# imaginateit/csm-train-pytorch

Measured on AMD Instinct MI355X. Metric: train tokens/sec (text+audio) CSM-1B bf16 seq2048, higher is better.
Workload: dtype bf16

## Files before the change

### csm-train-pytorch_amd/csm/engine.py

```python
from __future__ import annotations

import math
import numbers
from contextlib import contextmanager
from typing import Dict, List, Optional

import torch

from .hip import ops

BF16 = torch.bfloat16
F32 = torch.float32
import os as _os
FUSE_SWIGLU = _os.environ.get("CSM_FUSE_SWIGLU", "1") == "1"
FUSE_ROPE_BWD = _os.environ.get("CSM_FUSE_ROPE_BWD", "1") == "1"
FUSE_ROPE_FWD = _os.environ.get("CSM_FUSE_ROPE_FWD", "1") == "1"
PAIR_DX_DW = int(_os.environ.get("CSM_PAIR_DX_DW", "0"))
GROUP_ATTN_DW = _os.environ.get("CSM_GROUP_ATTN_DW", "1") == "1"
DEFER_ATTN_DW = int(_os.environ.get("CSM_DEFER_ATTN_DW", "3"))
DEFER_NORM_DW = _os.environ.get("CSM_DEFER_NORM_DW", "1") == "1"
ROWS_ON_HOST = _os.environ.get("CSM_ROWS_ON_HOST", "1") == "1"
EMB_KEYSORT = _os.environ.get("CSM_EMB_KEYSORT", "1") == "1"
DECODE_POS_HOST = _os.environ.get("CSM_DECODE_POS_HOST", "1") == "1"
LORA_FUSE = _os.environ.get("CSM_LORA_FUSE", "1") != "0"


def _refuse_stack(lo, where: str):
    if getattr(lo, "n_adapters", 1) > 1:
        raise ValueError(f"{where} takes one adapter set, and model.lora stacks {lo.n_adapters}: export one first "
                         "(state = model.lora.export(a), then LoRABank.add / generate_batch(adapters=[...]) / row_lora(model, state))")


def adapter_rows(adapter_ids, B: int, S: int, n_adapters: int, segment_lengths=None) -> torch.Tensor:
    ids = torch.as_tensor(adapter_ids).detach().to("cpu")
    if ids.is_floating_point() or ids.dtype == torch.bool:
        raise ValueError(f"adapter_ids must be integers, got {ids.dtype}")
    ids = ids.to(torch.int64)
# ... 650 lines not shown
        dh0 = self.backbone.backward(dhid, B, S, tr["backbone"], 1.0, on_layer_done=self.grad_hook, acc=acc["backbone"], seg=s.get("seg"),
                                    sel=s.get("sel"))
        if train_embeddings:
            self._embedding_backward(s, dh0, dseq if (dec is not None and s["aw"] != 0.0) else None)
        if self.grad_hook is not None:
            self.grad_hook("embeddings", -1)

    def _embedding_backward(self, s, dh0, dseq):
        m, a = self.m, self.m.args
        dev = m.device
        K, V = a.audio_num_codebooks, a.audio_vocab_size
        TV = a.text_vocab_size
        n_rows = TV + K * V
        tk, mk = s["tk"], s["mk"]
        M = tk.shape[0]
        ck = ("embbwd", M, K, V, TV)
        c = self._consts.get(ck)
        if c is None:
            slot = torch.arange(K + 1, device=dev)
            c = self._consts[ck] = dict(off=torch.where(slot < K, TV + slot * V, torch.zeros_like(slot)),
                                        src=torch.arange(M, device=dev).unsqueeze(1).expand(M, K + 1).reshape(-1).contiguous())
        rows = torch.where(mk.bool(), tk + c["off"], torch.full_like(tk, n_rows)).reshape(-1)
        src = c["src"]
        n_src = M
        if dseq is not None:
            codes, N = s["dec"]["codes"], s["dec"]["N"]
            dk = ("embbwd_dec", M, N, K, V, TV)
            d = self._consts.get(dk)
            if d is None:
                d = self._consts[dk] = dict(off=TV + torch.arange(K - 1, device=dev) * V,
                                            src=(M + torch.arange(N, device=dev).unsqueeze(1) * K + torch.arange(1, K, device=dev)).reshape(-1))
            rows = torch.cat([rows, (codes[:, :K - 1] + d["off"]).reshape(-1)])
            src = torch.cat([src, d["src"]])
            n_src = M + N * K
        if n_src <= (1 << 20) and EMB_KEYSORT:
            key = torch.sort((rows << 20) | src).values
            rows_s, src_s = key >> 20, key & ((1 << 20) - 1)
        else:
            order = torch.argsort(rows, stable=True)
            rows_s, src_s = rows[order].contiguous(), src[order].contiguous()
        ops.embed_bwd_sorted(rows_s, src_s, dh0, dseq,
                             m.block("text_embeddings.weight", True), m.block("audio_embeddings.weight", True))

    @torch.no_grad()
    def hidden_states(self, tokens: torch.Tensor, masks: torch.Tensor) -> torch.Tensor:
        m, a = self.m, self.m.args
        B, S, K1 = tokens.shape
        M = B * S
        tk = tokens.reshape(M, K1).to(device=m.device, dtype=torch.int64).contiguous()
        mk = masks.reshape(M, K1).to(device=m.device, dtype=torch.uint8).contiguous()
        h0 = torch.empty(M, m.bb.embed_dim, dtype=BF16, device=m.device)
        self._need()
        ops.embed_fwd(tk, mk, m.block("text_embeddings.weight"), m.block("audio_embeddings.weight"), h0, a.audio_vocab_size)
        return self.backbone.forward(h0, B, S, False).view(B, S, -1)

    @torch.no_grad()
    def generate_frame(self, tokens, tokens_mask, input_pos, temperature, topk, noise=None, adapters=None, top_p=None,
# ... 921 lines not shown
```

### csm-train-pytorch_amd/csm/hip/__init__.py

```python
import ctypes as C
import os

_HERE = os.path.dirname(os.path.abspath(__file__))
LIB_PATH = os.environ.get("CSM_HIP_LIB") or os.path.join(_HERE, "libcsm_hip.so")


class CsmHipError(RuntimeError):
    pass


if not os.path.exists(LIB_PATH):
    raise ImportError(
        f"{LIB_PATH} is missing: build it with `python __graft_entry__.py build` (or `make -C csm-train-pytorch_amd/csrc`). "
        "The CSM MI355X path has no fallback implementation."
    )

lib = C.CDLL(LIB_PATH)

_p, _i, _f, _ll = C.c_void_p, C.c_int, C.c_float, C.c_longlong

_SIGS = {
    "csm_abi_version": ([], _i),
    "csm_last_error": ([], C.c_char_p),
    "csm_device_check": ([_i], _i),
# ... 23 lines not shown
    "csm_colsum_rows_bf16": ([_p, _i, _ll, _i, _p, _i, _p], _i),
    "csm_rope": ([_p, _p, _p, _ll, _i, _i, _i, _i, _i, _p], _i),
    "csm_set_attn_variant": ([_i], _i),
    "csm_attn_last_dkv_kernel": ([], _i),
    "csm_attn64_set_debug": ([_p], _i),
    "csm_set_decode_tuning": ([_i, _i], _i),
    "csm_attn_fwd": ([_p, _p, _p, _i, _i, _i, _i, _i, _p], _i),
    "csm_attn_bwd": ([_p, _p, _p, _p, _p, _p, _i, _i, _i, _i, _i, _p], _i),
    "csm_attn_bwd_rope": ([_p, _p, _p, _p, _p, _p, _p, _i, _i, _i, _i, _i, _p], _i),
    "csm_attn_fwd_seg": ([_p, _p, _p, _p, _i, _i, _i, _i, _i, _p], _i),
    "csm_attn_bwd_seg": ([_p, _p, _p, _p, _p, _p, _p, _p, _i, _i, _i, _i, _i, _p], _i),
    "csm_swiglu_fwd": ([_p, _p, _ll, _i, _p], _i),
    "csm_swiglu_bwd": ([_p, _p, _p, _ll, _i, _p], _i),
    "csm_embed_fwd": ([_p, _p, _p, _p, _p, _ll, _i, _i, _i, _p], _i),
    "csm_embed_bwd_sorted": ([_p, _p, _ll, _p, _p, _ll, _p, _p, _ll, _ll, _i, _p], _i),
    "csm_rows_add_bf16": ([_p, _p, _p, _ll, _i, _i, _p], _i),
    "csm_rows_take_bf16": ([_p, _p, _p, _ll, _i, _p], _i),
    "csm_decoder_input_fwd": ([_p, _p, _p, _p, _p, _ll, _i, _i, _i, _p], _i),
    "csm_ce_fwd_bwd": ([_p, _p, _p, _p, _ll, _i, _i, _i, _f, _p], _i),
    "csm_reduce_sum_f32": ([_p, _ll, _f, _p, _p], _i),
    "csm_sumsq_blocks": ([], _i),
    "csm_sumsq_bf16": ([_p, _ll, _p, _p], _i),
    "csm_clip_coef": ([_p, _i, _f, _p, _p], _i),
    "csm_adamw_step": ([_p, _p, _p, _p, _p, _ll, _f, _f, _f, _f, _f, _i, _p, _f, _i, _p], _i),
    "csm_adamw_step_split": ([_p, _p, _p, _p, _p, _ll, _f, _f, _f, _f, _f, _i, _p, _f, _i, _p], _i),
    "csm_adamw_step_live": ([_p, _p, _p, _p, _p, _ll, _f, _f, _f, _f, _f, _i, _p, _f, _i, _p, _p], _i),
    "csm_adamw_step_split_live": ([_p, _p, _p, _p, _p, _ll, _f, _f, _f, _f, _f, _i, _p, _f, _i, _p, _p], _i),
    "csm_set_adamw_blocks": ([_i], _i),
    "csm_gemv_bf16": ([_p, _p, _p, _p, _i, _i, _i, _i, _i, _i, _i, _p], _i),
    "csm_gemv_last_kernel": ([], C.c_char_p),
# ... 82 lines not shown
```

### csm-train-pytorch_amd/csm/hip/ops.py

```python
import ctypes
import math
from typing import Optional

import torch

from . import CsmHipError, check, lib

BF16 = torch.bfloat16


def _stream() -> int:
    return torch.cuda.current_stream().cuda_stream


def _ptr(t: Optional[torch.Tensor]) -> Optional[int]:
    return None if t is None else t.data_ptr()


def _mat(t: torch.Tensor, dtype=BF16):
    assert t.is_cuda and t.dtype == dtype and t.dim() == 2 and t.stride(1) == 1, (t.dtype, t.shape, t.stride())
    return t.data_ptr(), t.shape[0], t.shape[1], t.stride(0)


def _pin(pin):
# ... 294 lines not shown

def swiglu_bwd(gu, dout, dgu):
    M, F2 = gu.shape
    check(lib.csm_swiglu_bwd(gu.data_ptr(), dout.data_ptr(), dgu.data_ptr(), M, F2 // 2, _stream()), "csm_swiglu_bwd")
    return dgu


def embed_fwd(tokens, mask_u8, text_emb, audio_emb, out, audio_vocab):
    M, K1 = tokens.shape
    assert tokens.dtype == torch.int64 and mask_u8.dtype == torch.uint8 and tokens.is_contiguous() and mask_u8.is_contiguous()
    check(lib.csm_embed_fwd(tokens.data_ptr(), mask_u8.data_ptr(), text_emb.data_ptr(), audio_emb.data_ptr(), out.data_ptr(),
                            M, K1 - 1, out.shape[1], audio_vocab, _stream()), "csm_embed_fwd")
    return out


def embed_bwd_sorted(sorted_rows, src_index, dh, dseq, g_text, g_audio):
    assert sorted_rows.dtype == torch.int64 and src_index.dtype == torch.int64 and sorted_rows.is_contiguous() and src_index.is_contiguous()
    check(lib.csm_embed_bwd_sorted(sorted_rows.data_ptr(), src_index.data_ptr(), sorted_rows.numel(), dh.data_ptr(), _ptr(dseq),
                                   dh.shape[0], g_text.data_ptr(), g_audio.data_ptr(), g_text.shape[0],
                                   g_text.shape[0] + g_audio.shape[0], dh.shape[1], _stream()), "csm_embed_bwd_sorted")


def rows_add_bf16(dst, rows_i32, src, src_stride_rows):
    check(lib.csm_rows_add_bf16(dst.data_ptr(), rows_i32.data_ptr(), src.data_ptr(), rows_i32.numel(), int(src_stride_rows),
                                dst.shape[1], _stream()), "csm_rows_add_bf16")


def rows_take_bf16(table, rows_i32, out):
    assert rows_i32.dtype == torch.int32 and rows_i32.is_contiguous() and out.is_contiguous() and out.shape == (rows_i32.numel(), table.shape[1])
    check(lib.csm_rows_take_bf16(table.data_ptr(), rows_i32.data_ptr(), out.data_ptr(), rows_i32.numel(), table.shape[1], _stream()),
# ... 13 lines not shown
    R, ldl = logits_f32.shape[0], logits_f32.stride(0)
    assert logits_f32.dtype == torch.float32 and targets.dtype == torch.int64 and targets.is_contiguous()
    ldd = dlogits.stride(0) if dlogits is not None else 0
    check(lib.csm_ce_fwd_bwd(logits_f32.data_ptr(), targets.data_ptr(), loss_rows.data_ptr(), _ptr(dlogits), R, V, ldl, ldd,
                             float(grad_scale), _stream()), "csm_ce_fwd_bwd")


def reduce_sum(x_f32, out_f32, scale=1.0):
    check(lib.csm_reduce_sum_f32(x_f32.data_ptr(), x_f32.numel(), float(scale), out_f32.data_ptr(), _stream()), "csm_reduce_sum_f32")


def sumsq_blocks() -> int:
    return lib.csm_sumsq_blocks()


def sumsq_bf16(g, partials):
    check(lib.csm_sumsq_bf16(g.data_ptr(), g.numel(), partials.data_ptr(), _stream()), "csm_sumsq_bf16")


def clip_coef(partials, max_norm, norm_and_coef):
    check(lib.csm_clip_coef(partials.data_ptr(), partials.numel(), float(max_norm), norm_and_coef.data_ptr(), _stream()), "csm_clip_coef")


ADAMW_BLOCK = 2048


def _live_ptr(block_live, n):
    assert block_live.dtype == torch.uint8 and block_live.is_contiguous() and block_live.numel() == -(-n // ADAMW_BLOCK)
    return block_live.data_ptr()


def adamw_step(master, m, v, param, grad, lr, beta1, beta2, eps, wd, step, norm_and_coef=None, grad_mul=1.0, zero_grad=False, *,
# ... 473 lines not shown
```

### csm-train-pytorch_amd/csm/models/model.py

```python
from __future__ import annotations

import math
from collections import OrderedDict
from dataclasses import dataclass
from typing import Dict, List, Optional, Tuple

import torch
import torch.nn as nn

from ..hip import ops, require_device

BF16 = torch.bfloat16


@dataclass
class StackConfig:
    embed_dim: int
    num_layers: int
    num_heads: int
    num_kv_heads: int
    intermediate_dim: int
    max_seq_len: int = 2048
    norm_eps: float = 1e-5
    rope_base: float = 500_000.0
# ... 143 lines not shown
        super().__init__()
        self.args = args
        self.bb: StackConfig = FLAVORS[args.backbone_flavor]()
        self.dc: StackConfig = FLAVORS[args.decoder_flavor]()
        self.vocab_pad = _pad64(args.audio_vocab_size)
        self._slots: Dict[str, _Slot] = OrderedDict()
        self._groups: Dict[str, Tuple[int, int]] = {}
        self._plan()
        self._device = torch.device("cpu")
        self.arena: Optional[torch.Tensor] = None
        self.grad_arena: Optional[torch.Tensor] = None
        self.lora = None
        self.acoustic_mode = "off"
        self.acoustic_fraction = 1.0 / 16.0
        self.grad_state = {"backbone": "zero", "decoder": "zero", "embeddings": "zero", "other": "zero"}
        self.target_ignore_index = None
        self._tables: Dict[str, torch.Tensor] = {}
        self._engine = None
        self._init_seed = seed
        self._fp32_source = None
        self.use_kv_cache = True
        self.use_hip_graph = True
        self._decode_weights = "bf16"
        self.trainable = {"backbone": True, "decoder": True, "embeddings": True, "other": True}
        if device is not None:
            self.to(device)

    @property
    def decode_weights(self) -> str:
        return self._decode_weights
# ... 69 lines not shown
        stack("decoder", self.dc)
        out["text_embeddings.weight"] = blk("text_embeddings.weight")
        out["audio_embeddings.weight"] = blk("audio_embeddings.weight")
        out["projection.weight"] = blk("projection.weight")
        out["codebook0_head.weight"] = blk("codebook0_head.padded")[:a.audio_vocab_size]
        out["audio_head"] = blk("audio_head.padded")[:, :, :a.audio_vocab_size]
        return out

    def block(self, name: str, grad: bool = False) -> torch.Tensor:
        s = self._slots[name]
        src = self.grad_arena if grad else self.arena
        return src[s.offset:s.offset + s.numel].view(s.shape)

    def group_range(self, group: str) -> Tuple[int, int]:
        return self._groups[group]

    def to(self, *args, **kwargs):
        device = kwargs.get("device", None)
        for a in args:
            if isinstance(a, (str, torch.device)):
                device = a
        if device is None:
            return self
        device = torch.device(device)
        if device.type != "cuda":
            raise RuntimeError("csm (MI355X build): the model lives on a gfx950 GPU; there is no CPU execution path")
        require_device(device.index or 0)
        if device.index is None:
            device = torch.device("cuda", torch.cuda.current_device())
        old = self.arena
        self.arena = torch.zeros(self._numel, dtype=BF16, device=device)
        if old is not None:
            self.arena.copy_(old)
        self.grad_arena = None
        self._device = device
        self._bind()
        if old is None:
            self.reset_parameters(self._init_seed)
        self._tables = {}
        self._engine = None
        return self

    def cuda(self, device=None):
        return self.to(torch.device("cuda", device if device is not None else torch.cuda.current_device()))

    def _bind(self):
        for name, view in self._views(self.arena).items():
            mod, _, leaf = name.rpartition(".")
            holder = self
# ... 123 lines not shown
```

### csm-train-pytorch_amd/csm/training/dp.py

```python
import os
from typing import Callable, Dict, List, Optional, Tuple

import torch
import torch.distributed as dist


def init_distributed(backend: Optional[str] = None) -> Tuple[int, int, int]:
    rank, world = int(os.environ.get("RANK", 0)), int(os.environ.get("WORLD_SIZE", 1))
    local = int(os.environ.get("LOCAL_RANK", 0))
    os.environ.setdefault("HSA_ENABLE_IPC_MODE_LEGACY", "0")
    if world > 1 and not dist.is_initialized():
        if torch.cuda.is_available():
            torch.cuda.set_device(local)
        backend = backend or ("nccl" if torch.cuda.is_available() else "gloo")
        if backend == "nccl":
            init_nccl(rank, world, local)
        else:
            dist.init_process_group(backend, rank=rank, world_size=world)
    return rank, world, local


def init_nccl(rank: int, world: int, local: int):
    kw = dict(rank=rank, world_size=world, device_id=torch.device("cuda", local))
    opts = None
# ... 98 lines not shown

    def attach(self):
        model, gs = self._model, self
        if gs.world_size > 1 and model.grad_arena.is_cuda and "CSM_GEMM256_PERSISTENT" not in os.environ \
                and self._restore_persistent is None:
            from ..hip import lib
            import logging
            gs._restore_persistent = lib.csm_get_gemm256_persistent()
            lib.csm_set_gemm256_persistent(0)
            logging.getLogger("csm_trainer").info(
                "data parallel: 256x256 GEMM switched from persistent workgroups to one tile per workgroup while gradient "
                "collectives share the CUs (CSM_GEMM256_PERSISTENT pins it; GradSync.close() restores the previous setting)")
        model.engine.grad_hook = gs.on_ready
        if self.zero1:
            model.engine.param_hook = gs.wait_params

    def close(self):
        self.check_overflow(block=True)
        m = getattr(self, "_model", None)
        if m is not None and getattr(m.engine, "grad_hook", None) == self.on_ready:
            m.engine.grad_hook = None
        if self.zero1:
            self.wait_params(None, None)
            if m is not None and getattr(m.engine, "param_hook", None) == self.wait_params:
                m.engine.param_hook = None
        if self._restore_persistent is not None:
            from ..hip import lib
            lib.csm_set_gemm256_persistent(self._restore_persistent)
            self._restore_persistent = None

    @staticmethod
    def _merge(slices: List[Tuple[int, int]]) -> List[Tuple[int, int]]:
        out: List[Tuple[int, int]] = []
        for off, n in sorted(slices):
            if out and off - (out[-1][0] + out[-1][1]) < 64:
                out[-1] = (out[-1][0], off + n - out[-1][0])
# ... 295 lines not shown
```

### csm-train-pytorch_amd/csm/training/optim.py

```python
import os
from typing import Dict, List, Optional

import torch

from ..hip import ops

F32 = torch.float32
SPLIT_MASTER = os.environ.get("CSM_ADAMW_SPLIT", "1") == "1"
FLAGGED_GROUPS = ("embeddings",)


def split_master(master: torch.Tensor, param_out: torch.Tensor) -> torch.Tensor:
    bits = master.contiguous().view(torch.int32)
    param_out.view(torch.int16).copy_(((bits + 0x8000) >> 16).to(torch.int16))
    return (bits & 0xFFFF).to(torch.int16)


def join_master(param: torch.Tensor, lo: torch.Tensor) -> torch.Tensor:
    hi = param.view(torch.int16).to(torch.int32) & 0xFFFF
    l = lo.to(torch.int32) & 0xFFFF
    return (((hi - (l >> 15)) << 16) | l).view(torch.float32)


def seed_master(model, offset: int, numel: int, param: torch.Tensor, from_fp32_source: bool = False) -> torch.Tensor:
# ... 53 lines not shown
                                          param=model.arena[off:off + n], grad=model.grad_arena[off:off + n]))
        if model.lora is not None and lora_lr is not None:
            lo = model.lora
            self.param_groups.append(dict(name="lora", lr=float(lora_lr), weight_decay=lora_weight_decay, offset=0,
                                          numel=lo.arena.numel(), param=lo.arena, grad=lo.grad_arena))
        for g in self.param_groups:
            master = self._seed_master(g, from_fp32_source=True)
            if SPLIT_MASTER:
                lo = split_master(master, g["param"])
                self.state[g["name"]] = dict(lo=lo, m=torch.zeros_like(master), v=torch.zeros_like(master))
                del master
            else:
                self.state[g["name"]] = dict(master=master, m=torch.zeros_like(master), v=torch.zeros_like(master))
            if self.dead_blocks and g["name"] in FLAGGED_GROUPS:
                self.state[g["name"]]["live"] = torch.zeros(-(-g["numel"] // ops.ADAMW_BLOCK), dtype=torch.uint8, device=g["param"].device)
        self._partials = torch.empty(max(1, len(self.param_groups)) * ops.sumsq_blocks(), dtype=F32, device=model.device)
        self._norm_coef = torch.ones(2, dtype=F32, device=model.device)
        import weakref
        if not hasattr(model, "_optimizers"):
            model._optimizers = []
        model._optimizers.append(weakref.ref(self))

    def _seed_master(self, g, from_fp32_source: bool = False) -> torch.Tensor:
        return seed_master(self.model, g["offset"], g["numel"], g["param"], from_fp32_source and g["name"] != "lora")

    def moments_rewritten(self):
        for name in FLAGGED_GROUPS:
            if self.dead_blocks and name in self.state:
                st = self.state[name]
                st["live"] = live_blocks(st["m"], st["v"])

    def named_master(self):
        m = self.model
        views, base = m._views(m.arena), m.arena.storage_offset()
        for g in self.param_groups:
            if g["name"] == "lora":
                continue
            master = self.master(g["name"])
            for k, v in views.items():
                so = v.storage_offset() - base
                if g["offset"] <= so < g["offset"] + g["numel"]:
                    yield k, torch.as_strided(master, v.size(), v.stride(), so - g["offset"])

    def _group(self, name):
        return next(g for g in self.param_groups if g["name"] == name)
# ... 4 lines not shown

    def set_master(self, name: str, master: torch.Tensor):
        st, g = self.state[name], self._group(name)
        if "master" in st:
            st["master"].copy_(master)
            g["param"].copy_(st["master"])
        else:
            st["lo"].copy_(split_master(master.to(device=g["param"].device, dtype=F32), g["param"]))

    def num_trainable(self) -> int:
        return sum(g["numel"] for g in self.param_groups)

    def zero_grad(self, set_to_none: bool = False):
        for g in self.param_groups:
            g["grad"].zero_()
            if g["name"] in self.model.grad_state:
                self.model.grad_state[g["name"]] = "zero"
        self._coef = None

    def _settle(self):
        gs = self.model.grad_state
        for g in self.param_groups:
            if gs.get(g["name"]) == "stale":
                g["grad"].zero_()
                gs[g["name"]] = "zero"

    def clip_grad_norm(self, max_norm: float) -> torch.Tensor:
        self._settle()
        nb = ops.sumsq_blocks()
        for i, g in enumerate(self.param_groups):
            ops.sumsq_bf16(g["grad"], self._partials[i * nb:(i + 1) * nb])
        ops.clip_coef(self._partials[:len(self.param_groups) * nb], max_norm, self._norm_coef)
        self._coef = self._norm_coef
        return self._norm_coef[0]

    def step(self, zero_grad=False, skip: Optional[torch.Tensor] = None):
        self._settle()
        self.step_count += 1
        self.model._fp32_source = None
        if skip is not None:
            coef = self._coef[1] if self._coef is not None else torch.ones((), dtype=F32, device=skip.device)
            self._norm_coef[1] = torch.where(skip.reshape(()) != 0, torch.full_like(coef, -1.0), coef)
            self._coef = self._norm_coef
        b1, b2 = self.betas
        gs = self.model.grad_state
        for g in self.param_groups:
            st = self.state[g["name"]]
            name = g["name"]
            zero = bool(zero_grad) if zero_grad != "lazy" else (name == "embeddings" or name not in gs)
            if "lo" in st:
                ops.adamw_step_split(st["lo"], st["m"], st["v"], g["param"], g["grad"], g["lr"], b1, b2, self.eps,
                                     g["weight_decay"], self.step_count, self._coef, zero_grad=zero, block_live=st.get("live"))
            else:
                ops.adamw_step(st["master"], st["m"], st["v"], g["param"], g["grad"], g["lr"], b1, b2, self.eps,
                               g["weight_decay"], self.step_count, self._coef, zero_grad=zero, block_live=st.get("live"))
            if name in gs:
                if zero:
                    gs[name] = "zero"
                elif zero_grad == "lazy" and gs[name] == "live":
                    gs[name] = "stale"
        self._coef = None

    def uncount_step(self):
        self.step_count = max(0, self.step_count - 1)

    def params_rewritten(self, base: bool = True, lora: bool = True, from_fp32_source: bool = False):
        for g in self.param_groups:
            if lora if g["name"] == "lora" else base:
                self.set_master(g["name"], self._seed_master(g, from_fp32_source))

# ... 8 lines not shown
        if sorted(saved_by_name) != sorted(mine) or sorted(sd["state"]) != sorted(mine):
            raise ValueError(f"optimizer state was saved for parameter groups {sorted(saved_by_name)} but this optimizer has "
                             f"{sorted(mine)} (different freeze flags / LoRA setting?)")
        for g in self.param_groups:
            saved = saved_by_name[g["name"]]
            if (saved["offset"], saved["numel"]) != (g["offset"], g["numel"]):
                raise ValueError(f"optimizer group {g['name']!r}: saved range {saved['offset']}+{saved['numel']} != {g['offset']}+{g['numel']}")
        self.step_count = sd["step"]
        for n, st in sd["state"].items():
            for k, v in st.items():
                if k == "master":
                    self.set_master(n, v)
                else:
                    self.state[n][k].copy_(v)
        self.moments_rewritten()
        for g in self.param_groups:
            saved = saved_by_name[g["name"]]
            g["lr"], g["weight_decay"] = saved["lr"], saved["weight_decay"]
```

### csm-train-pytorch_amd/csrc/ops.hip

```cpp
#include "common.h"
#include <math.h>

namespace {

template <int NC>
__global__ __launch_bounds__(256) void rmsnorm_fwd_kernel(const bf16_t* __restrict__ x, const bf16_t* __restrict__ w,
                                                          bf16_t* __restrict__ y, float* __restrict__ rstd, int M, int D,
                                                          float eps) {
    const int lane = threadIdx.x & 63;
    const int wpb = blockDim.x >> 6;
    const int nchunk = D >> 3;
    for (long long row = (long long)blockIdx.x * wpb + (threadIdx.x >> 6); row < M; row += (long long)gridDim.x * wpb) {
        U4 v[NC];
        float ss = 0.f;
#pragma unroll
        for (int i = 0; i < NC; ++i) {
            const int c = lane + 64 * i;
            v[i] = (U4){0u, 0u, 0u, 0u};
            if (c < nchunk) v[i] = *reinterpret_cast<const U4*>(x + (size_t)row * D + c * 8);
            float f[8];
            unpack8(v[i], f);
#pragma unroll
            for (int j = 0; j < 8; ++j) ss += f[j] * f[j];
        }
// ... 285 lines not shown
    const uint8_t* mk = mask + row * (K + 1);
    for (int c0 = threadIdx.x * 8; c0 < D; c0 += blockDim.x * 8) {
        float acc[8] = {0.f, 0.f, 0.f, 0.f, 0.f, 0.f, 0.f, 0.f};
        for (int s = 0; s <= K; ++s) {
            if (!mk[s]) continue;
            const bf16_t* src = (s < K) ? audio_emb + ((size_t)tok[s] + (size_t)s * audio_vocab) * D : text_emb + (size_t)tok[s] * D;
            float f[8];
            unpack8(*reinterpret_cast<const U4*>(src + c0), f);
#pragma unroll
            for (int j = 0; j < 8; ++j) acc[j] += f[j];
        }
        *reinterpret_cast<U4*>(out + (size_t)row * D + c0) = pack8(acc);
    }
}

template <int NC>
__global__ __launch_bounds__(256) void embed_bwd_sorted_kernel(const long long* __restrict__ rows, const long long* __restrict__ src,
                                                               long long n_occ, const bf16_t* __restrict__ dh,
                                                               const bf16_t* __restrict__ dseq, long long M,
                                                               bf16_t* __restrict__ g_text, bf16_t* __restrict__ g_audio,
                                                               long long text_rows, long long n_rows, int D) {
    const int lane = threadIdx.x & 63;
    const long long i = (long long)blockIdx.x * (blockDim.x >> 6) + (threadIdx.x >> 6);
    if (i >= n_occ) return;
    const long long r = rows[i];
    if (r >= n_rows || (i > 0 && rows[i - 1] == r)) return;
    float acc[NC][8];
#pragma unroll
    for (int c = 0; c < NC; ++c)
#pragma unroll
        for (int j = 0; j < 8; ++j) acc[c][j] = 0.f;
    const int nchunk = D >> 3;
    for (long long k = i; k < n_occ && rows[k] == r; ++k) {
        const long long sidx = src[k];
        const bf16_t* p = sidx < M ? dh + (size_t)sidx * D : dseq + (size_t)(sidx - M) * D;
#pragma unroll
        for (int c = 0; c < NC; ++c) {
            const int ch = lane + 64 * c;
            if (ch < nchunk) {
                float f[8];
                unpack8(*reinterpret_cast<const U4*>(p + ch * 8), f);
#pragma unroll
                for (int j = 0; j < 8; ++j) acc[c][j] += f[j];
            }
        }
    }
    bf16_t* dst = r < text_rows ? g_text + (size_t)r * D : g_audio + (size_t)(r - text_rows) * D;
#pragma unroll
    for (int c = 0; c < NC; ++c) {
        const int ch = lane + 64 * c;
        if (ch < nchunk) {
            float f[8];
            unpack8(*reinterpret_cast<const U4*>(dst + ch * 8), f);
#pragma unroll
            for (int j = 0; j < 8; ++j) f[j] += acc[c][j];
            *reinterpret_cast<U4*>(dst + ch * 8) = pack8(f);
        }
    }
}

// ... 148 lines not shown
#pragma unroll
        for (int j = 0; j < 8; ++j) acc += f1[j] * f1[j];
#pragma unroll
        for (int j = 0; j < 8; ++j) acc += f2[j] * f2[j];
#pragma unroll
        for (int j = 0; j < 8; ++j) acc += f3[j] * f3[j];
    }
    for (; i < nvec; i += stride) {
        float f[8];
        unpack8(*reinterpret_cast<const U4*>(g + i * 8), f);
#pragma unroll
        for (int j = 0; j < 8; ++j) acc += f[j] * f[j];
    }
    if (blockIdx.x == 0)
        for (long long i = (nvec << 3) + threadIdx.x; i < n; i += blockDim.x) { const float f = bf2f(g[i]); acc += f * f; }
    acc = block_sum(acc, red);
    if (threadIdx.x == 0) partials[blockIdx.x] = acc;
}

__global__ __launch_bounds__(1024) void clip_coef_kernel(const float* __restrict__ partials, int n, float max_norm,
                                                         float* __restrict__ out) {
    __shared__ float red[16];
    float acc = 0.f;
    for (int i = threadIdx.x; i < n; i += blockDim.x) acc += partials[i];
    acc = block_sum(acc, red);
    if (threadIdx.x == 0) {
        const float norm = sqrtf(acc);
        out[0] = norm;
        out[1] = (max_norm > 0.f) ? fminf(1.f, max_norm / (norm + 1e-6f)) : 1.f;
    }
// ... 336 lines not shown
extern "C" int csm_embed_bwd_sorted(const long long* sorted_rows, const long long* src_index, long long n_occ, const void* dh,
                                    const void* dseq, long long M, void* g_text, void* g_audio, long long text_rows,
                                    long long n_rows, int D, hipStream_t stream) {
    CSM_REQUIRE(sorted_rows && src_index && dh && g_text && g_audio && n_occ > 0, "csm_embed_bwd_sorted: bad arguments");
    CSM_REQUIRE((D & 7) == 0 && D <= 4096, "csm_embed_bwd_sorted: D=%d must be a multiple of 8 and <= 4096", D);
    const long long blocks = (n_occ + 3) / 4;
    CSM_REQUIRE(blocks < (1ll << 31), "csm_embed_bwd_sorted: too many occurrences");
    const int nc = (D + 511) / 512;
#define L(NC) hipLaunchKernelGGL((embed_bwd_sorted_kernel<NC>), dim3((unsigned)blocks), dim3(256), 0, stream, sorted_rows, src_index, n_occ, (const bf16_t*)dh, (const bf16_t*)dseq, M, (bf16_t*)g_text, (bf16_t*)g_audio, text_rows, n_rows, D)
    if (nc <= 1) L(1); else if (nc <= 2) L(2); else if (nc <= 4) L(4); else L(8);
#undef L
    CSM_CHECK_LAUNCH("csm_embed_bwd_sorted");
    return 0;
}

extern "C" int csm_rows_add_bf16(void* dst, const int* rows, const void* src, long long N, int src_stride_rows, int D,
                                 hipStream_t stream) {
    CSM_REQUIRE(dst && rows && src && N > 0 && (D & 7) == 0 && src_stride_rows > 0, "csm_rows_add_bf16: bad arguments");
    hipLaunchKernelGGL(rows_add_kernel, dim3((unsigned)((N + 3) / 4)), dim3(256), 0, stream, (bf16_t*)dst, rows, (const bf16_t*)src,
                       N, src_stride_rows, D);
    CSM_CHECK_LAUNCH("csm_rows_add_bf16");
    return 0;
}

extern "C" int csm_rows_take_bf16(void* table, const int* rows, void* out, long long N, int D, hipStream_t stream) {
    CSM_REQUIRE(table && rows && out && N > 0 && (D & 7) == 0, "csm_rows_take_bf16: bad arguments");
    hipLaunchKernelGGL(rows_take_kernel, dim3((unsigned)((N + 3) / 4)), dim3(256), 0, stream, (bf16_t*)table, rows, (bf16_t*)out, N, D);
    CSM_CHECK_LAUNCH("csm_rows_take_bf16");
    return 0;
}
// ... 32 lines not shown
    hipLaunchKernelGGL(reduce_sum_kernel, dim3(1), dim3(1024), 0, stream, x, n, scale, out);
    CSM_CHECK_LAUNCH("csm_reduce_sum_f32");
    return 0;
}

#define CSM_SUMSQ_BLOCKS 8192
extern "C" int csm_sumsq_blocks(void) { return CSM_SUMSQ_BLOCKS; }

extern "C" int csm_sumsq_bf16(const void* g, long long n, float* partials, hipStream_t stream) {
    CSM_REQUIRE(g && partials && n > 0 && ((uintptr_t)g & 15) == 0, "csm_sumsq_bf16: bad arguments");
    hipLaunchKernelGGL(sumsq_kernel, dim3(CSM_SUMSQ_BLOCKS), dim3(256), 0, stream, (const bf16_t*)g, n, partials);
    CSM_CHECK_LAUNCH("csm_sumsq_bf16");
    return 0;
}

extern "C" int csm_clip_coef(const float* partials, int n_partials, float max_norm, float* norm_and_coef,
                             hipStream_t stream) {
    CSM_REQUIRE(partials && norm_and_coef && n_partials > 0, "csm_clip_coef: bad arguments");
    hipLaunchKernelGGL(clip_coef_kernel, dim3(1), dim3(1024), 0, stream, partials, n_partials, max_norm, norm_and_coef);
    CSM_CHECK_LAUNCH("csm_clip_coef");
    return 0;
}

static int g_adamw_blocks = 1 << 20;
extern "C" int csm_set_adamw_blocks(int b) { g_adamw_blocks = b; return 0; }

extern "C" int csm_adamw_step(float* master, float* m, float* v, void* param, void* grad, long long n, float lr,
                              float beta1, float beta2, float eps, float weight_decay, int step,
                              const float* norm_and_coef, float grad_mul, int zero_grad, hipStream_t stream) {
    CSM_REQUIRE(master && m && v && param && grad && n > 0 && step > 0, "csm_adamw_step: bad arguments");
// ... 51 lines not shown
```

### include/csm_hip.h

```cpp
#ifndef CSM_HIP_H
#define CSM_HIP_H
#include <stdint.h>

#ifdef __cplusplus
extern "C" {
#endif

typedef struct ihipStream_t* csm_stream_t;

int csm_abi_version(void);
const char* csm_last_error(void);
int csm_device_check(int device);

int csm_gemm_bf16(const void* A, const void* B, void* C, const void* R, int M, int N, int K, int lda, int ldb, int ldc,
                  int ldr, int transA, int transB, int out_f32, float alpha, int batch, long long strideA,
                  long long strideB, long long strideC, long long strideR, csm_stream_t stream);

int csm_gemm_bf16_ex(const void* A, const void* B, void* C, const void* R, int M, int N, int K, int lda, int ldb, int ldc,
                     int ldr, int transA, int transB, int out_f32, float alpha, int batch, long long strideA,
                     long long strideB, long long strideC, long long strideR, int epilogue, const void* aux_in,
                     void* aux_out, int ld_aux, csm_stream_t stream);
int csm_gemm_bf16_rope(const void* A, const void* W, void* C, int M, int N, int K, int lda, int ldw, int ldc,
                       const float* rope_table, int rows_per_seq, int n_rope_cols, int head_dim, csm_stream_t stream);
int csm_gemm_bf16_kext(const void* A, const void* B, void* C, const void* R, int M, int N, int K, int lda, int ldb, int ldc, int ldr,
// ... 49 lines not shown
int csm_attn_last_dkv_kernel(void);
int csm_attn_fwd_seg(const void* qkv, void* out, float* lse, const int* seg_start, int B, int S, int H, int KV, int HD, csm_stream_t stream);
int csm_attn_bwd_seg(const void* qkv, const void* out, const void* dout, const float* lse, void* dqkv, float* delta_ws,
                     const int* seg_start, const int* seg_end, int B, int S, int H, int KV, int HD, csm_stream_t stream);
int csm_attn64_set_debug(void* device_buffer);

int csm_swiglu_fwd(const void* gu, void* out, long long M, int F, csm_stream_t stream);
int csm_swiglu_bwd(const void* gu, const void* dout, void* dgu, long long M, int F, csm_stream_t stream);

int csm_embed_fwd(const long long* tokens, const uint8_t* mask, const void* text_emb, const void* audio_emb, void* out,
                  long long M, int K, int D, int audio_vocab, csm_stream_t stream);

int csm_embed_bwd_sorted(const long long* sorted_rows, const long long* src_index, long long n_occ, const void* dh,
                         const void* dseq, long long M, void* g_text, void* g_audio, long long text_rows, long long n_rows,
                         int D, csm_stream_t stream);
int csm_rows_add_bf16(void* dst, const int* rows, const void* src, long long N, int src_stride_rows, int D, csm_stream_t stream);
int csm_rows_take_bf16(void* table, const int* rows, void* out, long long N, int D, csm_stream_t stream);

int csm_decoder_input_fwd(const void* hidden, const int* rows, const long long* codes, const void* audio_emb, void* out,
                          long long N, int K, int D, int audio_vocab, csm_stream_t stream);

int csm_ce_fwd_bwd(const float* logits, const long long* targets, float* loss_rows, void* dlogits, long long R, int V,
                   int ldl, int ldd, float grad_scale, csm_stream_t stream);
int csm_reduce_sum_f32(const float* x, long long n, float scale, float* out, csm_stream_t stream);

int csm_sumsq_blocks(void);
int csm_sumsq_bf16(const void* g, long long n, float* partials , csm_stream_t stream);
int csm_clip_coef(const float* partials, int n_partials, float max_norm, float* norm_and_coef , csm_stream_t stream);
int csm_adamw_step(float* master, float* m, float* v, void* param, void* grad, long long n, float lr, float beta1,
                   float beta2, float eps, float weight_decay, int step, const float* norm_and_coef ,
// ... 124 lines not shown
```

Measured before the change: 133,500.

## Build embedding sort keys natively and skip untouched gradient blocks in norm

```diff
diff --git a/csm-train-pytorch_amd/csm/engine.py b/csm-train-pytorch_amd/csm/engine.py
--- a/csm-train-pytorch_amd/csm/engine.py
+++ b/csm-train-pytorch_amd/csm/engine.py
@@ -21,6 +21,7 @@
 DEFER_NORM_DW = _os.environ.get("CSM_DEFER_NORM_DW", "1") == "1"
 ROWS_ON_HOST = _os.environ.get("CSM_ROWS_ON_HOST", "1") == "1"
 EMB_KEYSORT = _os.environ.get("CSM_EMB_KEYSORT", "1") == "1"
+EMB_NATIVE_KEYS = _os.environ.get("CSM_EMB_NATIVE_KEYS", "1") == "1"
 DECODE_POS_HOST = _os.environ.get("CSM_DECODE_POS_HOST", "1") == "1"
 LORA_FUSE = _os.environ.get("CSM_LORA_FUSE", "1") != "0"
 
@@ -701,6 +702,15 @@
         n_rows = TV + K * V
         tk, mk = s["tk"], s["mk"]
         M = tk.shape[0]
+        g_text, g_audio = m.block("text_embeddings.weight", True), m.block("audio_embeddings.weight", True)
+        if EMB_KEYSORT and EMB_NATIVE_KEYS and M + (s["dec"]["N"] * K if dseq is not None else 0) <= (1 << 20):
+            keys = ops.embed_keys(tk, mk, s["dec"]["codes"] if dseq is not None else None, V, TV)
+            g0 = m.group_range("embeddings")[0]
+            ops.embed_bwd_keys(torch.sort(keys).values, dh0, dseq, g_text, g_audio, flags=m.grad_flags(),
+                               text_base=m._slots["text_embeddings.weight"].offset - g0,
+                               audio_base=m._slots["audio_embeddings.weight"].offset - g0)
+            return
+        m.grads_rewritten()
         ck = ("embbwd", M, K, V, TV)
         c = self._consts.get(ck)
         if c is None:
@@ -726,8 +736,7 @@
         else:
             order = torch.argsort(rows, stable=True)
             rows_s, src_s = rows[order].contiguous(), src[order].contiguous()
-        ops.embed_bwd_sorted(rows_s, src_s, dh0, dseq,
-                             m.block("text_embeddings.weight", True), m.block("audio_embeddings.weight", True))
+        ops.embed_bwd_sorted(rows_s, src_s, dh0, dseq, g_text, g_audio)
 
     @torch.no_grad()
     def hidden_states(self, tokens: torch.Tensor, masks: torch.Tensor) -> torch.Tensor:
diff --git a/csm-train-pytorch_amd/csm/hip/__init__.py b/csm-train-pytorch_amd/csm/hip/__init__.py
--- a/csm-train-pytorch_amd/csm/hip/__init__.py
+++ b/csm-train-pytorch_amd/csm/hip/__init__.py
@@ -61,6 +61,9 @@
     "csm_swiglu_bwd": ([_p, _p, _p, _ll, _i, _p], _i),
     "csm_embed_fwd": ([_p, _p, _p, _p, _p, _ll, _i, _i, _i, _p], _i),
     "csm_embed_bwd_sorted": ([_p, _p, _ll, _p, _p, _ll, _p, _p, _ll, _ll, _i, _p], _i),
+    "csm_embed_keys": ([_p, _p, _p, _p, _ll, _ll, _i, _i, _ll, _p], _i),
+    "csm_embed_bwd_keys": ([_p, _ll, _p, _p, _ll, _p, _p, _ll, _ll, _i, _p, _ll, _ll, _ll, _p], _i),
+    "csm_sumsq_bf16_flagged": ([_p, _ll, _p, _p, _p], _i),
     "csm_rows_add_bf16": ([_p, _p, _p, _ll, _i, _i, _p], _i),
     "csm_rows_take_bf16": ([_p, _p, _p, _ll, _i, _p], _i),
     "csm_decoder_input_fwd": ([_p, _p, _p, _p, _p, _ll, _i, _i, _i, _p], _i),
diff --git a/csm-train-pytorch_amd/csm/hip/ops.py b/csm-train-pytorch_amd/csm/hip/ops.py
--- a/csm-train-pytorch_amd/csm/hip/ops.py
+++ b/csm-train-pytorch_amd/csm/hip/ops.py
@@ -332,6 +332,29 @@
     return out
 
 
+def embed_keys(tokens, mask_u8, codes, audio_vocab, text_rows):
+    M, K1 = tokens.shape
+    assert tokens.dtype == torch.int64 and mask_u8.dtype == torch.uint8 and tokens.is_contiguous() and mask_u8.is_contiguous()
+    assert mask_u8.shape == tokens.shape
+    N = 0
+    if codes is not None:
+        assert codes.dtype == torch.int64 and codes.is_contiguous() and codes.shape[1] == K1 - 1
+        N = codes.shape[0]
+    keys = torch.empty(M * K1 + N * (K1 - 2), dtype=torch.int64, device=tokens.device)
+    check(lib.csm_embed_keys(tokens.data_ptr(), mask_u8.data_ptr(), _ptr(codes), keys.data_ptr(), M, N, K1 - 1, audio_vocab,
+                             text_rows, _stream()), "csm_embed_keys")
+    return keys
+
+
+def embed_bwd_keys(sorted_keys, dh, dseq, g_text, g_audio, *, flags=None, text_base=0, audio_base=0):
+    assert sorted_keys.dtype == torch.int64 and sorted_keys.is_contiguous()
+    assert flags is None or (flags.dtype == torch.uint8 and flags.is_contiguous())
+    check(lib.csm_embed_bwd_keys(sorted_keys.data_ptr(), sorted_keys.numel(), dh.data_ptr(), _ptr(dseq), dh.shape[0],
+                                 g_text.data_ptr(), g_audio.data_ptr(), g_text.shape[0], g_text.shape[0] + g_audio.shape[0],
+                                 dh.shape[1], _ptr(flags),
+                                 0 if flags is None else flags.numel(), int(text_base), int(audio_base), _stream()), "csm_embed_bwd_keys")
+
+
 def embed_bwd_sorted(sorted_rows, src_index, dh, dseq, g_text, g_audio):
     assert sorted_rows.dtype == torch.int64 and src_index.dtype == torch.int64 and sorted_rows.is_contiguous() and src_index.is_contiguous()
     check(lib.csm_embed_bwd_sorted(sorted_rows.data_ptr(), src_index.data_ptr(), sorted_rows.numel(), dh.data_ptr(), _ptr(dseq),
@@ -375,8 +398,12 @@
     return lib.csm_sumsq_blocks()
 
 
-def sumsq_bf16(g, partials):
-    check(lib.csm_sumsq_bf16(g.data_ptr(), g.numel(), partials.data_ptr(), _stream()), "csm_sumsq_bf16")
+def sumsq_bf16(g, partials, *, flags=None):
+    if flags is None:
+        check(lib.csm_sumsq_bf16(g.data_ptr(), g.numel(), partials.data_ptr(), _stream()), "csm_sumsq_bf16")
+    else:
+        check(lib.csm_sumsq_bf16_flagged(g.data_ptr(), g.numel(), partials.data_ptr(), _live_ptr(flags, g.numel()), _stream()),
+              "csm_sumsq_bf16_flagged")
 
 
 def clip_coef(partials, max_norm, norm_and_coef):
diff --git a/csm-train-pytorch_amd/csm/models/model.py b/csm-train-pytorch_amd/csm/models/model.py
--- a/csm-train-pytorch_amd/csm/models/model.py
+++ b/csm-train-pytorch_amd/csm/models/model.py
@@ -1,6 +1,7 @@
 from __future__ import annotations
 
 import math
+import os
 from collections import OrderedDict
 from dataclasses import dataclass
 from typing import Dict, List, Optional, Tuple
@@ -181,6 +182,8 @@
         self.acoustic_mode = "off"
         self.acoustic_fraction = 1.0 / 16.0
         self.grad_state = {"backbone": "zero", "decoder": "zero", "embeddings": "zero", "other": "zero"}
+        self.emb_grad_flags: Optional[torch.Tensor] = None
+        self._grad_flags_off = False
         self.target_ignore_index = None
         self._tables: Dict[str, torch.Tensor] = {}
         self._engine = None
@@ -280,6 +283,22 @@
 
     def group_range(self, group: str) -> Tuple[int, int]:
         return self._groups[group]
+
+    def grad_flags(self, create: bool = False) -> Optional[torch.Tensor]:
+        if self._grad_flags_off or os.environ.get("CSM_EMB_GRAD_FLAGS", "1") != "1":
+            return None
+        if self.emb_grad_flags is None and create and self.grad_arena is not None:
+            n = self.group_range("embeddings")[1]
+            self.emb_grad_flags = torch.ones(-(-n // 2048), dtype=torch.uint8, device=self.grad_arena.device)
+        return self.emb_grad_flags
+
+    def grads_rewritten(self):
+        if self.emb_grad_flags is not None:
+            self.emb_grad_flags.fill_(1)
+
+    def set_grad_flags_off(self, off: bool):
+        self._grad_flags_off = bool(off)
+        self.grads_rewritten()
 
     def to(self, *args, **kwargs):
         device = kwargs.get("device", None)
@@ -299,6 +318,7 @@
         if old is not None:
             self.arena.copy_(old)
         self.grad_arena = None
+        self.emb_grad_flags = None
         self._device = device
         self._bind()
         if old is None:
diff --git a/csm-train-pytorch_amd/csm/training/dp.py b/csm-train-pytorch_amd/csm/training/dp.py
--- a/csm-train-pytorch_amd/csm/training/dp.py
+++ b/csm-train-pytorch_amd/csm/training/dp.py
@@ -136,12 +136,14 @@
         model.engine.grad_hook = gs.on_ready
         if self.zero1:
             model.engine.param_hook = gs.wait_params
+        model.set_grad_flags_off(True)
 
     def close(self):
         self.check_overflow(block=True)
         m = getattr(self, "_model", None)
         if m is not None and getattr(m.engine, "grad_hook", None) == self.on_ready:
             m.engine.grad_hook = None
+            m.set_grad_flags_off(False)
         if self.zero1:
             self.wait_params(None, None)
             if m is not None and getattr(m.engine, "param_hook", None) == self.wait_params:
diff --git a/csm-train-pytorch_amd/csm/training/optim.py b/csm-train-pytorch_amd/csm/training/optim.py
--- a/csm-train-pytorch_amd/csm/training/optim.py
+++ b/csm-train-pytorch_amd/csm/training/optim.py
@@ -91,6 +91,8 @@
                 self.state[g["name"]] = dict(master=master, m=torch.zeros_like(master), v=torch.zeros_like(master))
             if self.dead_blocks and g["name"] in FLAGGED_GROUPS:
                 self.state[g["name"]]["live"] = torch.zeros(-(-g["numel"] // ops.ADAMW_BLOCK), dtype=torch.uint8, device=g["param"].device)
+            if g["name"] == "embeddings":
+                model.grad_flags(create=True)
         self._partials = torch.empty(max(1, len(self.param_groups)) * ops.sumsq_blocks(), dtype=F32, device=model.device)
         self._norm_coef = torch.ones(2, dtype=F32, device=model.device)
         import weakref
@@ -106,6 +108,19 @@
             if self.dead_blocks and name in self.state:
                 st = self.state[name]
                 st["live"] = live_blocks(st["m"], st["v"])
+
+    def grads_rewritten(self):
+        model = getattr(self, "model", None)
+        if model is not None:
+            model.grads_rewritten()
+
+    def _grad_flags(self, g) -> Optional[torch.Tensor]:
+        return self.model.grad_flags() if g["name"] == "embeddings" and not self.sharded else None
+
+    def _zeroed(self, g):
+        flags = self._grad_flags(g)
+        if flags is not None:
+            flags.zero_()
 
     def named_master(self):
         m = self.model
@@ -140,6 +155,7 @@
     def zero_grad(self, set_to_none: bool = False):
         for g in self.param_groups:
             g["grad"].zero_()
+            self._zeroed(g)
             if g["name"] in self.model.grad_state:
                 self.model.grad_state[g["name"]] = "zero"
         self._coef = None
@@ -149,13 +165,14 @@
         for g in self.param_groups:
             if gs.get(g["name"]) == "stale":
                 g["grad"].zero_()
+                self._zeroed(g)
                 gs[g["name"]] = "zero"
 
     def clip_grad_norm(self, max_norm: float) -> torch.Tensor:
         self._settle()
         nb = ops.sumsq_blocks()
         for i, g in enumerate(self.param_groups):
-            ops.sumsq_bf16(g["grad"], self._partials[i * nb:(i + 1) * nb])
+            ops.sumsq_bf16(g["grad"], self._partials[i * nb:(i + 1) * nb], flags=self._grad_flags(g))
         ops.clip_coef(self._partials[:len(self.param_groups) * nb], max_norm, self._norm_coef)
         self._coef = self._norm_coef
         return self._norm_coef[0]
@@ -180,6 +197,8 @@
             else:
                 ops.adamw_step(st["master"], st["m"], st["v"], g["param"], g["grad"], g["lr"], b1, b2, self.eps,
                                g["weight_decay"], self.step_count, self._coef, zero_grad=zero, block_live=st.get("live"))
+            if zero:
+                self._zeroed(g)
             if name in gs:
                 if zero:
                     gs[name] = "zero"
@@ -218,6 +237,7 @@
                 else:
                     self.state[n][k].copy_(v)
         self.moments_rewritten()
+        self.grads_rewritten()
         for g in self.param_groups:
             saved = saved_by_name[g["name"]]
             g["lr"], g["weight_decay"] = saved["lr"], saved["weight_decay"]
diff --git a/csm-train-pytorch_amd/csrc/ops.hip b/csm-train-pytorch_amd/csrc/ops.hip
--- a/csm-train-pytorch_amd/csrc/ops.hip
+++ b/csm-train-pytorch_amd/csrc/ops.hip
@@ -323,6 +323,27 @@
     }
 }
 
+__global__ __launch_bounds__(256) void embed_keys_kernel(const long long* __restrict__ tokens, const uint8_t* __restrict__ mask,
+                                                         const long long* __restrict__ codes, long long* __restrict__ keys,
+                                                         long long M, long long N, int K, int audio_vocab, long long text_rows) {
+    const long long n1 = M * (K + 1), n = n1 + (codes ? N * (K - 1) : 0);
+    const long long n_rows = text_rows + (long long)K * audio_vocab;
+    for (long long e = (long long)blockIdx.x * blockDim.x + threadIdx.x; e < n; e += (long long)gridDim.x * blockDim.x) {
+        long long row, src;
+        if (e < n1) {
+            src = e / (K + 1);
+            const int s = (int)(e - src * (K + 1));
+            row = mask[e] ? tokens[e] + (s < K ? text_rows + (long long)s * audio_vocab : 0) : n_rows;
+        } else {
+            const long long e2 = e - n1, f = e2 / (K - 1);
+            const int j = (int)(e2 - f * (K - 1));
+            row = codes[f * K + j] + text_rows + (long long)j * audio_vocab;
+            src = M + f * K + j + 1;
+        }
+        keys[e] = (row << 20) | src;
+    }
+}
+
 template <int NC>
 __global__ __launch_bounds__(256) void embed_bwd_sorted_kernel(const long long* __restrict__ rows, const long long* __restrict__ src,
                                                                long long n_occ, const bf16_t* __restrict__ dh,
@@ -353,6 +374,56 @@
                 for (int j = 0; j < 8; ++j) acc[c][j] += f[j];
             }
         }
+    }
+    bf16_t* dst = r < text_rows ? g_text + (size_t)r * D : g_audio + (size_t)(r - text_rows) * D;
+#pragma unroll
+    for (int c = 0; c < NC; ++c) {
+        const int ch = lane + 64 * c;
+        if (ch < nchunk) {
+            float f[8];
+            unpack8(*reinterpret_cast<const U4*>(dst + ch * 8), f);
+#pragma unroll
+            for (int j = 0; j < 8; ++j) f[j] += acc[c][j];
+            *reinterpret_cast<U4*>(dst + ch * 8) = pack8(f);
+        }
+    }
+}
+
+template <int NC>
+__global__ __launch_bounds__(256) void embed_bwd_keys_kernel(const long long* __restrict__ keys, long long n_occ,
+                                                             const bf16_t* __restrict__ dh, const bf16_t* __restrict__ dseq, long long M,
+                                                             bf16_t* __restrict__ g_text, bf16_t* __restrict__ g_audio,
+                                                             long long text_rows, long long n_rows, int D,
+                                                             uint8_t* __restrict__ flags, long long text_base, long long audio_base) {
+    constexpr long long SRC = (1ll << 20) - 1;
+    const int lane = threadIdx.x & 63;
+    const long long i = (long long)blockIdx.x * (blockDim.x >> 6) + (threadIdx.x >> 6);
+    if (i >= n_occ) return;
+    const long long r = keys[i] >> 20;
+    if (r >= n_rows || (i > 0 && (keys[i - 1] >> 20) == r)) return;
+    float acc[NC][8];
+#pragma unroll
+    for (int c = 0; c < NC; ++c)
+#pragma unroll
+        for (int j = 0; j < 8; ++j) acc[c][j] = 0.f;
+    const int nchunk = D >> 3;
+    for (long long k = i; k < n_occ && (keys[k] >> 20) == r; ++k) {
+        const long long sidx = keys[k] & SRC;
+        const bf16_t* p = sidx < M ? dh + (size_t)sidx * D : dseq + (size_t)(sidx - M) * D;
+#pragma unroll
+        for (int c = 0; c < NC; ++c) {
+            const int ch = lane + 64 * c;
+            if (ch < nchunk) {
+                float f[8];
+                unpack8(*reinterpret_cast<const U4*>(p + ch * 8), f);
+#pragma unroll
+                for (int j = 0; j < 8; ++j) acc[c][j] += f[j];
+            }
+        }
+    }
+    if (flags) {
+        const long long e0 = r < text_rows ? text_base + r * D : audio_base + (r - text_rows) * D;
+        for (long long b = (e0 >> 11) + lane; b <= ((e0 + D - 1) >> 11); b += 64) flags[b] = 1;
     }
     bf16_t* dst = r < text_rows ? g_text + (size_t)r * D : g_audio + (size_t)(r - text_rows) * D;
 #pragma unroll
@@ -531,6 +602,44 @@
     }
     if (blockIdx.x == 0)
         for (long long i = (nvec << 3) + threadIdx.x; i < n; i += blockDim.x) { const float f = bf2f(g[i]); acc += f * f; }
+    acc = block_sum(acc, red);
+    if (threadIdx.x == 0) partials[blockIdx.x] = acc;
+}
+
+__global__ __launch_bounds__(256) void sumsq_flagged_kernel(const bf16_t* __restrict__ g, long long n, float* __restrict__ partials,
+                                                            const uint8_t* __restrict__ flags) {
+    __shared__ float red[16];
+    float acc = 0.f;
+    const long long nvec = n >> 3;
+    const long long stride = (long long)gridDim.x * blockDim.x;
+    long long i = (long long)blockIdx.x * blockDim.x + threadIdx.x;
+    const U4 zero = {0u, 0u, 0u, 0u};
+    for (; i + 3 * stride < nvec; i += 4 * stride) {
+        const uint8_t w0 = flags[i >> 8], w1 = flags[(i + stride) >> 8], w2 = flags[(i + 2 * stride) >> 8], w3 = flags[(i + 3 * stride) >> 8];
+        if (!(w0 | w1 | w2 | w3)) continue;
+        const U4 q0 = w0 ? *reinterpret_cast<const U4*>(g + i * 8) : zero, q1 = w1 ? *reinterpret_cast<const U4*>(g + (i + stride) * 8) : zero;
+        const U4 q2 = w2 ? *reinterpret_cast<const U4*>(g + (i + 2 * stride) * 8) : zero, q3 = w3 ? *reinterpret_cast<const U4*>(g + (i + 3 * stride) * 8) : zero;
+        float f0[8], f1[8], f2[8], f3[8];
+        unpack8(q0, f0); unpack8(q1, f1); unpack8(q2, f2); unpack8(q3, f3);
+#pragma unroll
+        for (int j = 0; j < 8; ++j) acc += f0[j] * f0[j];
+#pragma unroll
+        for (int j = 0; j < 8; ++j) acc += f1[j] * f1[j];
+#pragma unroll
+        for (int j = 0; j < 8; ++j) acc += f2[j] * f2[j];
+#pragma unroll
+        for (int j = 0; j < 8; ++j) acc += f3[j] * f3[j];
+    }
+    for (; i < nvec; i += stride) {
+        if (!flags[i >> 8]) continue;
+        float f[8];
+        unpack8(*reinterpret_cast<const U4*>(g + i * 8), f);
+#pragma unroll
+        for (int j = 0; j < 8; ++j) acc += f[j] * f[j];
+    }
+    if (blockIdx.x == 0)
+        for (long long i = (nvec << 3) + threadIdx.x; i < n; i += blockDim.x)
+            if (flags[i >> 11]) { const float f = bf2f(g[i]); acc += f * f; }
     acc = block_sum(acc, red);
     if (threadIdx.x == 0) partials[blockIdx.x] = acc;
 }
@@ -897,6 +1006,37 @@
     return 0;
 }
 
+extern "C" int csm_embed_keys(const long long* tokens, const uint8_t* mask, const long long* codes, long long* keys, long long M,
+                              long long N, int K, int audio_vocab, long long text_rows, hipStream_t stream) {
+    CSM_REQUIRE(tokens && mask && keys && M > 0 && K > 0 && audio_vocab > 0 && text_rows >= 0, "csm_embed_keys: bad arguments");
+    CSM_REQUIRE(!codes || (N > 0 && K > 1), "csm_embed_keys: codes need N > 0 and K > 1");
+    CSM_REQUIRE(M + (codes ? N * K : 0) <= (1ll << 20), "csm_embed_keys: more than 2^20 gradient source rows");
+    const long long n = M * (K + 1) + (codes ? N * (K - 1) : 0);
+    hipLaunchKernelGGL(embed_keys_kernel, dim3(grid_for(n, 256, 4096)), dim3(256), 0, stream, tokens, mask, codes, keys, M, N, K,
+                       audio_vocab, text_rows);
+    CSM_CHECK_LAUNCH("csm_embed_keys");
+    return 0;
+}
+
+extern "C" int csm_embed_bwd_keys(const long long* sorted_keys, long long n_occ, const void* dh, const void* dseq, long long M,
+                                  void* g_text, void* g_audio, long long text_rows, long long n_rows, int D,
+                                  void* flags, long long n_flags, long long text_base, long long audio_base, hipStream_t stream) {
+    CSM_REQUIRE(sorted_keys && dh && g_text && g_audio && n_occ > 0, "csm_embed_bwd_keys: bad arguments");
+    CSM_REQUIRE(!flags || (text_base >= 0 && audio_base >= 0 && text_rows <= n_rows &&
+                           ((text_base + text_rows * D + 2047) >> 11) <= n_flags &&
+                           ((audio_base + (n_rows - text_rows) * D + 2047) >> 11) <= n_flags),
+                "csm_embed_bwd_keys: the tables do not fit %lld flag blocks", n_flags);
+    CSM_REQUIRE((D & 7) == 0 && D <= 4096, "csm_embed_bwd_keys: D=%d must be a multiple of 8 and <= 4096", D);
+    const long long blocks = (n_occ + 3) / 4;
+    CSM_REQUIRE(blocks < (1ll << 31), "csm_embed_bwd_keys: too many occurrences");
+    const int nc = (D + 511) / 512;
+#define L(NC) hipLaunchKernelGGL((embed_bwd_keys_kernel<NC>), dim3((unsigned)blocks), dim3(256), 0, stream, sorted_keys, n_occ, (const bf16_t*)dh, (const bf16_t*)dseq, M, (bf16_t*)g_text, (bf16_t*)g_audio, text_rows, n_rows, D, (uint8_t*)flags, text_base, audio_base)
+    if (nc <= 1) L(1); else if (nc <= 2) L(2); else if (nc <= 4) L(4); else L(8);
+#undef L
+    CSM_CHECK_LAUNCH("csm_embed_bwd_keys");
+    return 0;
+}
+
 extern "C" int csm_rows_add_bf16(void* dst, const int* rows, const void* src, long long N, int src_stride_rows, int D,
                                  hipStream_t stream) {
     CSM_REQUIRE(dst && rows && src && N > 0 && (D & 7) == 0 && src_stride_rows > 0, "csm_rows_add_bf16: bad arguments");
@@ -959,6 +1099,14 @@
     return 0;
 }
 
+extern "C" int csm_sumsq_bf16_flagged(const void* g, long long n, float* partials, const void* flags, hipStream_t stream) {
+    CSM_REQUIRE(g && partials && flags && n > 0 && ((uintptr_t)g & 15) == 0, "csm_sumsq_bf16_flagged: bad arguments");
+    hipLaunchKernelGGL(sumsq_flagged_kernel, dim3(CSM_SUMSQ_BLOCKS), dim3(256), 0, stream, (const bf16_t*)g, n, partials,
+                       (const uint8_t*)flags);
+    CSM_CHECK_LAUNCH("csm_sumsq_bf16_flagged");
+    return 0;
+}
+
 extern "C" int csm_clip_coef(const float* partials, int n_partials, float max_norm, float* norm_and_coef,
                              hipStream_t stream) {
     CSM_REQUIRE(partials && norm_and_coef && n_partials > 0, "csm_clip_coef: bad arguments");
diff --git a/include/csm_hip.h b/include/csm_hip.h
--- a/include/csm_hip.h
+++ b/include/csm_hip.h
@@ -87,6 +87,12 @@
 int csm_embed_bwd_sorted(const long long* sorted_rows, const long long* src_index, long long n_occ, const void* dh,
                          const void* dseq, long long M, void* g_text, void* g_audio, long long text_rows, long long n_rows,
                          int D, csm_stream_t stream);
+int csm_embed_keys(const long long* tokens, const uint8_t* mask, const long long* codes, long long* keys, long long M,
+                   long long N, int K, int audio_vocab, long long text_rows, csm_stream_t stream);
+int csm_embed_bwd_keys(const long long* sorted_keys, long long n_occ, const void* dh, const void* dseq, long long M,
+                       void* g_text, void* g_audio, long long text_rows, long long n_rows, int D,
+                       void* flags, long long n_flags, long long text_base, long long audio_base, csm_stream_t stream);
+int csm_sumsq_bf16_flagged(const void* g, long long n, float* partials, const void* flags, csm_stream_t stream);
 int csm_rows_add_bf16(void* dst, const int* rows, const void* src, long long N, int src_stride_rows, int D, csm_stream_t stream);
 int csm_rows_take_bf16(void* table, const int* rows, void* out, long long N, int D, csm_stream_t stream);
 
```

Result: no change. 133,900 (median of 6 runs) (+0.3%).
